# titus-leistner/mmlf

Measured on AMD Instinct MI355X. Metric: 96x96 EPI patches/sec fwd+bwd, bs=512, higher is better.
Workload: dtype f32 via 2 x f16 operand split (22 significant bits per operand, locally scaled; 3 MFMA passes, f32 accumulate)

## Files before the change

### include/mmlf_hip.h

```cpp
#ifndef MMLF_HIP_H
#define MMLF_HIP_H

#include <stddef.h>
#include <stdint.h>

#ifdef __cplusplus
extern "C" {
#endif

#define MMLF_TILE_POSITIONS 256

const char *mmlf_last_error(void);
#define MMLF_ABI_VERSION 10
int mmlf_abi_version(void);

const char *mmlf_build_info(void);
int mmlf_build_is_ablation(void);
int mmlf_conv_cus(void);

enum { MMLF_AUDIT_IN = 0, MMLF_AUDIT_PACKED = 1, MMLF_AUDIT_BIAS = 2, MMLF_AUDIT_OUT = 3, MMLF_AUDIT_REF = 4,
       MMLF_AUDIT_IN_AMAX = 5, MMLF_AUDIT_OUT_AMAX = 6, MMLF_AUDIT_BN_PARTIAL = 7, MMLF_AUDIT_MASK = 8, MMLF_AUDIT_CONV_N = 9 };
int mmlf_audit_conv_h2(int cs_in, int K, int N, int cs_out, int N_store, int out_shift, int cs_ref, int B, int H, int W,
                       int64_t *ends);
enum { MMLF_AUDIT_WG_IN = 0, MMLF_AUDIT_WG_G = 1, MMLF_AUDIT_WG_GW = 2, MMLF_AUDIT_WG_GB = 3, MMLF_AUDIT_WG_WORKSPACE = 4,
       MMLF_AUDIT_WG_IN_AMAX = 5, MMLF_AUDIT_WG_G_AMAX = 6, MMLF_AUDIT_WGRAD_N = 7 };
int mmlf_audit_wgrad_h2(int cs_in, int Cin, int cs_g, int Cout, int g_shift, int B, int H, int W, int64_t *ends);

int64_t mmlf_grid_alloc_positions(int B, int H, int W);
int64_t mmlf_packed_filter_floats(int K, int N);
int64_t mmlf_wgrad_workspace_floats(int Cin, int Cout, int B, int H, int W);

enum { MMLF_VAR_IDENTITY = 0, MMLF_VAR_TRANSPOSE = 1, MMLF_VAR_TRANSPOSE_FLIPH = 2 };

int mmlf_pack_filter(const float *w_oihw, float *packed, int Cout, int Cin, int variant, int dgrad,
                     void *stream);

// ... 63 lines not shown
                        const float *running_var, double eps, float *scale, float *shift, int C,
                        void *stream);
int mmlf_fold_bn_eval(const float *w_oihw, const float *bias, const float *scale, const float *shift,
                      float *w_out, float *bias_out, int Cout, int Cin, void *stream);
int mmlf_bn_stats_finalize(const double *partial, int nblocks, int C, const float *gamma, const float *beta,
                           float *running_mean, float *running_var, double momentum, double eps,
                           float *save_mean, float *save_invstd, float *scale, float *shift,
                           int B, int H, int W, void *stream);
int mmlf_bn_apply_relu(const float *z, int cs_z, int C, const float *scale, const float *shift,
                       float *y, int cs_y, int c_off, int C_store, int B, int H, int W,
                       float *amax_out , void *stream);
int mmlf_bn_apply_relu4(const float *const z[4], int cs_z, int C, const float *const scale[4],
                        const float *const shift[4], float *y, int cs_y, int B, int H, int W,
                        float *amax_out , void *stream);
int mmlf_bn_bwd_reduce(const float *gy, int cs_gy, int c_off, const float *z, int cs_z, int C,
                       const float *scale, const float *shift, const float *gamma,
                       const float *save_mean, const float *save_invstd,
                       float *dgamma, float *dbeta, int accumulate, float *coef,
                       double *partial, int nblocks, int B, int H, int W, void *stream);
int mmlf_bn_bwd_apply(const float *gy, int cs_gy, int c_off, const float *z, int cs_z, int C,
                      const float *scale, const float *shift, const float *save_mean,
                      const float *coef, float *dz, int cs_dz, int B, int H, int W,
                      float *amax_out , void *stream);
int mmlf_relu_bwd_slice(const float *src, int cs_src, int c_off, const float *ref, int cs_ref, int ref_off, int C,
                        float *dst, int cs_dst, int B, int H, int W,
                        float *amax_out , void *stream);
enum { MMLF_AUDIT_SLICE_SRC = 0, MMLF_AUDIT_SLICE_REF = 1, MMLF_AUDIT_SLICE_DST = 2, MMLF_AUDIT_SLICE_AMAX = 3,
       MMLF_AUDIT_SLICE_N = 4 };
int mmlf_audit_relu_bwd_slice(int cs_src, int c_off, int cs_ref, int ref_off, int C, int cs_dst, int B, int H, int W,
                              int64_t *ends);

int mmlf_pack_nchw(const float *nchw, int C, float *grid, int cs, int B, int H, int W,
                   float *amax_out , void *stream);
int mmlf_unpack_nchw(const float *grid, int cs, float *nchw, int C, int B, int H, int W, void *stream);
int mmlf_zero_slack(float *grid, int cs, int B, int H, int W, float *amax, void *stream);
int mmlf_zero_slack4(float *const grid[4], const int cs[4], float *const amax[4], int B, int H, int W, void *stream);

int64_t mmlf_grid_alloc_positions_k3(int B, int H, int W);
int mmlf_zero_slack_k3(float *grid, int cs, int B, int H, int W, float *amax, void *stream);
int mmlf_zero_slack4_k3(float *const grid[4], const int cs[4], float *const amax[4], int B, int H, int W, void *stream);
int64_t mmlf_packed_filter3x3_floats(int K, int N);
int mmlf_pack_filter3x3(const float *w_oihw, float *packed, int Cout, int Cin, int variant, int dgrad, void *stream);
int mmlf_conv3x3(const float *in, int cs_in, int K, const float *packed, const float *bias, int N,
                 float *out, int cs_out, int N_store, int B, int H, int W, int relu, const float *relu_ref, int cs_ref,
                 void *stream);
int64_t mmlf_wgrad3x3_workspace_floats(int Cin, int Cout, int B, int H, int W);
// ... 56 lines not shown
```

### mmlf_amd/_lib.py

```python
import ctypes
import os

_HERE = os.path.dirname(os.path.abspath(__file__))
LIB_PATH = os.environ.get('MMLF_HIP_LIB') or os.path.join(_HERE, 'csrc', 'libmmlf_hip.so')

_vp = ctypes.c_void_p
_i = ctypes.c_int
_i64 = ctypes.c_int64
_d = ctypes.c_double

SIGNATURES = {
    'mmlf_last_error': (ctypes.c_char_p, []),
    'mmlf_abi_version': (_i, []),
    'mmlf_build_info': (ctypes.c_char_p, []),
    'mmlf_build_is_ablation': (_i, []),
    'mmlf_conv_cus': (_i, []),
    'mmlf_audit_conv_h2': (_i, [_i] * 10 + [_vp]),
    'mmlf_audit_wgrad_h2': (_i, [_i] * 8 + [_vp]),
    'mmlf_grid_alloc_positions': (_i64, [_i, _i, _i]),
    'mmlf_packed_filter_floats': (_i64, [_i, _i]),
    'mmlf_wgrad_workspace_floats': (_i64, [_i, _i, _i, _i, _i]),
    'mmlf_pack_filter': (_i, [_vp, _vp, _i, _i, _i, _i, _vp]),
    'mmlf_conv2x2': (_i, [_vp, _i, _i, _vp, _vp, _i, _vp, _i, _i, _i, _i, _i, _i, _i, _i, _i, _vp, _i, _vp]),
    'mmlf_packed_filter_split_bytes': (_i64, [_i, _i]),
# ... 6 lines not shown
    'mmlf_grid_pad_h': (_i, []),
    'mmlf_amax_head': (_i, []),
    'mmlf_amax_shard_stride': (_i, []),
    'mmlf_pack_filter_h2': (_i, [_vp, _vp, _i, _i, _i, _i, _vp]),
    'mmlf_packed_filter_h2_columns': (_i, [_i]),
    'mmlf_pack_filters_h2': (_i, [_vp, _i, _i, _vp]),
    'mmlf_conv2x2_h2': (_i, [_vp, _i, _i, _vp, _vp, _i, _vp, _i, _i, _i, _i, _i, _i, _i, _i, _i, _vp, _i, _vp, _vp, _vp, _vp, _vp, _vp]),
    'mmlf_relu_mask_words': (_i64, [_i, _i, _i]),
    'mmlf_conv2x2_thin_workspace_floats': (_i64, [_i, _i, _i]),
    'mmlf_conv2x2_thin': (_i, [_vp, _i, _i, _vp, _vp, _i, _vp, _i, _i, _i, _i, _i, _i, _i, _i, _i, _vp, _vp, _vp]),
    'mmlf_conv2x2_wgrad_thin_workspace_floats': (_i64, [_i]),
    'mmlf_conv2x2_wgrad_thin': (_i, [_vp, _i, _i, _vp, _i, _i, _i, _vp, _vp, _i, _i, _vp, _i, _i, _i, _vp]),
    'mmlf_conv2x2_blocks': (_i, [_i, _i, _i, _i, _i]),
    'mmlf_bn_stats_finalize': (_i, [_vp, _i, _i, _vp, _vp, _vp, _vp, _d, _d, _vp, _vp, _vp, _vp, _i, _i, _i, _vp]),
    'mmlf_conv2x2_wgrad': (_i, [_vp, _i, _i, _vp, _i, _i, _i, _vp, _vp, _i, _i, _vp, _i, _i, _i, _vp]),
    'mmlf_conv2x2_wgrad_split': (_i, [_vp, _i, _i, _vp, _i, _i, _i, _vp, _vp, _i, _i, _vp, _i, _i, _i, _vp]),
    'mmlf_bn_stats_train': (_i, [_vp, _i, _i, _vp, _vp, _vp, _vp, _d, _d, _vp, _vp, _vp, _vp, _vp, _i, _i, _i, _i, _vp]),
    'mmlf_bn_coeffs_eval': (_i, [_vp, _vp, _vp, _vp, _d, _vp, _vp, _i, _vp]),
    'mmlf_fold_bn_eval': (_i, [_vp, _vp, _vp, _vp, _vp, _vp, _i, _i, _vp]),
    'mmlf_bn_apply_relu': (_i, [_vp, _i, _i, _vp, _vp, _vp, _i, _i, _i, _i, _i, _i, _vp, _vp]),
    'mmlf_bn_apply_relu4': (_i, [_vp, _i, _i, _vp, _vp, _vp, _i, _i, _i, _i, _vp, _vp]),
    'mmlf_bn_bwd_reduce': (_i, [_vp, _i, _i, _vp, _i, _i, _vp, _vp, _vp, _vp, _vp, _vp, _vp, _i, _vp, _vp, _i, _i, _i, _i, _vp]),
    'mmlf_bn_bwd_apply': (_i, [_vp, _i, _i, _vp, _i, _i, _vp, _vp, _vp, _vp, _vp, _i, _i, _i, _i, _vp, _vp]),
    'mmlf_relu_bwd_slice': (_i, [_vp, _i, _i, _vp, _i, _i, _i, _vp, _i, _i, _i, _i, _vp, _vp]),
    'mmlf_audit_relu_bwd_slice': (_i, [_i] * 9 + [_vp]),
    'mmlf_pack_nchw': (_i, [_vp, _i, _vp, _i, _i, _i, _i, _vp, _vp]),
    'mmlf_zero_slack': (_i, [_vp, _i, _i, _i, _i, _vp, _vp]),
    'mmlf_zero_slack4': (_i, [_vp, _vp, _vp, _i, _i, _i, _vp]),
    'mmlf_unpack_nchw': (_i, [_vp, _i, _vp, _i, _i, _i, _i, _vp]),
    'mmlf_head_upr': (_i, [_vp, _vp, _vp, _i, _i, _i, _i, _vp]),
    'mmlf_head_dpp': (_i, [_vp, _vp, _vp, _vp, _vp, _vp, _vp, _i, _i, _i, _i, _vp]),
    'mmlf_head_upr_bwd': (_i, [_vp, _vp, _vp, _vp, _i, _i, _i, _i, _vp]),
    'mmlf_head_dpp_bwd': (_i, [_vp, _vp, _vp, _vp, _vp, _vp, _i, _i, _i, _i, _vp]),
    'mmlf_loss_fwd_bwd': (_i, [_i, _vp, _i, _vp, _vp, _vp, _d, _vp, _vp, _vp, _i, _vp, _i, _i, _i, _vp]),
    'mmlf_loss_multi_scratch_doubles': (_i64, [_i]),
    'mmlf_loss_multi_fwd_bwd': (_i, [_i, _vp, _i, _vp, _i, _vp, _vp, _vp, _d, _vp, _vp, _vp, _i, _vp, _vp, _i, _i, _i, _vp]),
    'mmlf_adam_step': (_i, [_vp, _vp, _vp, _vp, _i64, _d, _d, _d, _d, _i64, _d, _vp]),
    'mmlf_shift_views': (_i, [_vp, _vp, _vp, _vp, _vp, _vp, _vp, _vp, _vp, _vp, _i, _i, _i, _i, _vp]),
    'mmlf_shift_pack': (_i, [_vp, _i, _vp, _i, _vp, _vp, _i, _i, _i, _i, _vp, _vp]),
    'mmlf_lmm_to_discrete': (_i, [_vp, _vp, _vp, _vp, _i, _i, _i, _i64, _vp]),
    'mmlf_patch_gather': (_i, [_vp] * 5 + [_i] * 5 + [_vp] * 12 + [_i, _i, _vp]),
    'mmlf_patch_contrast': (_i, [_vp, _vp, _vp, _vp, _i, _i, _i, _vp]),
    'mmlf_ensamble_reduce': (_i, [_vp, _vp, _vp, _vp, _vp, _vp, _i, _i, _i, _i, _vp]),
    'mmlf_grid_alloc_positions_k3': (_i64, [_i, _i, _i]),
    'mmlf_zero_slack_k3': (_i, [_vp, _i, _i, _i, _i, _vp, _vp]),
    'mmlf_zero_slack4_k3': (_i, [_vp, _vp, _vp, _i, _i, _i, _vp]),
# ... 85 lines not shown
```

### mmlf_amd/csrc/common.h

```cpp
#pragma once
#include <hip/hip_runtime.h>
#include <stdint.h>
#include <stdio.h>
#include <stdarg.h>
#include <mutex>

#define MMLF_TILE 256
#define MMLF_TILE_MAX 512

extern thread_local char g_mmlf_err[512];

static inline int mmlf_fail(const char *fmt, ...)
{
    va_list ap;
    va_start(ap, fmt);
    vsnprintf(g_mmlf_err, sizeof(g_mmlf_err), fmt, ap);
    va_end(ap);
    return 1;
}

#define MMLF_CHECK_ARG(cond, ...)                   \
    do {                                            \
        if (!(cond)) return mmlf_fail(__VA_ARGS__); \
    } while (0)

static inline int mmlf_launch_status(const char *what)
{
    hipError_t e = hipGetLastError();
    if (e != hipSuccess) return mmlf_fail("%s: launch failed: %s", what, hipGetErrorString(e));
    return 0;
}

static inline int current_device()
{
    int d = 0;
    if (hipGetDevice(&d) != hipSuccess || d < 0 || d >= 64) d = 0;
    return d;
}
struct PerDeviceOnce {
    std::once_flag flag[64];
    int status[64] = {};
    template <class F> int run(F &&f)
    {
        const int d = current_device();
        std::call_once(flag[d], [&] { status[d] = f(); });
        return status[d];
    }
};
static inline int mmlf_allow_lds(const void *kernel, size_t bytes, const char *what)
{
    const hipError_t e = hipFuncSetAttribute(kernel, hipFuncAttributeMaxDynamicSharedMemorySize, (int)bytes);
    if (e != hipSuccess)
        return mmlf_fail("%s: hipFuncSetAttribute(MaxDynamicSharedMemorySize = %zu) failed: %s", what, bytes, hipGetErrorString(e));
    return 0;
// ... 99 lines not shown
```

### mmlf_amd/csrc/elementwise.hip

```cpp
#include "common.h"
#include "../../include/mmlf_hip.h"

thread_local char g_mmlf_err[512] = "";

extern "C" const char *mmlf_last_error(void) { return g_mmlf_err; }
extern "C" int mmlf_abi_version(void) { return MMLF_ABI_VERSION; }
extern "C" int64_t mmlf_amax_entries(int B, int H, int W)
{
    if (B <= 0 || H <= 0 || W <= 0) return -1;
    return amax_entries(make_grid(B, H, W));
}
extern "C" int mmlf_grid_pad_w(void) { return GRID_PAD; }
extern "C" int mmlf_grid_pad_h(void) { return GRID_PAD; }
extern "C" int mmlf_amax_head(void) { return MMLF_AMAX_HEAD; }
extern "C" int mmlf_amax_shard_stride(void) { return MMLF_AMAX_SHARD_STRIDE; }
extern "C" int64_t mmlf_grid_alloc_positions(int B, int H, int W)
{
    if (B <= 0 || H <= 0 || W <= 0) return -1;
    return grid_alloc_positions(make_grid(B, H, W));
}
extern "C" int64_t mmlf_grid_alloc_positions_k3(int B, int H, int W)
{
    if (B <= 0 || H <= 0 || W <= 0) return -1;
    return grid_alloc_positions_k3(make_grid(B, H, W));
// ... 286 lines not shown
            for (int k = 0; k < V; ++k) {
                const int c = V * cg + k;
                const float u = fmaf(zz[k], coefs[c], coefs[Cpad + c]);
                if (MODE == 0) {
                    o[k] = fmaxf(u, 0.f);
                } else {
                    const float g = u > 0.f ? gg[k] : 0.f;
                    o[k] = coefs[3 * Cpad + c] * g - coefs[4 * Cpad + c] - coefs[5 * Cpad + c] * (zz[k] - coefs[2 * Cpad + c]);
                }
            }
        }
#pragma unroll
        for (int k = 0; k < V; ++k) mx = fmaxf(mx, fabsf(o[k]));
        float *op = out + (base + x) * cs_out + c_off_out + V * cg;
        if (V * cg + V - 1 < C_store) {
            VecIO<V>::store_nt(op, o);
        } else {
#pragma unroll
            for (int k = 0; k < V; ++k)
                if (V * cg + k < C_store) op[k] = o[k];
        }
    }
    if (amax) mmlf_amax_update_row(mx, amax, row);
    }
}

template <int V>
__global__ __launch_bounds__(256) void relu_slice_rows_kernel(const float *__restrict__ src, int cs_src, int c_off,
                                                              const float *__restrict__ ref, int cs_ref, int ref_off, int C,
                                                              float *__restrict__ dst, int cs_dst, int H, int W,
                                                              float *__restrict__ amax, int nrows)
{
    const int P = W + GRID_PAD, R = H + GRID_PAD;
    const int cvn = cs_dst / V;
    const int dx = 256 / cvn, dc = 256 - dx * cvn;
    for (int row = blockIdx.x; row < nrows; row += gridDim.x) {
        const int y = row % R;
        const size_t base = (size_t)row * P;
        const bool row_in = (y >= 1 && y <= H);
        int x = threadIdx.x / cvn, cg = threadIdx.x - x * cvn;
        float mx = 0.f;
        for (; x < P; x += dx, cg += dc) {
            if (cg >= cvn) { cg -= cvn; ++x; if (x >= P) break; }
            float o[V];
#pragma unroll
            for (int k = 0; k < V; ++k) o[k] = 0.f;
// ... 996 lines not shown
    hipStream_t st = (hipStream_t)stream;
    hipLaunchKernelGGL(bn_reduce_bwd_kernel, dim3(nblocks), dim3(256), 0, st, z, cs_z, gy, cs_gy, c_off,
                       scale, shift, save_mean, save_invstd, C, partial, B, H, W);
    hipLaunchKernelGGL(bn_bwd_finalize_kernel, dim3(C), dim3(64), 0, st, partial, nblocks, C,
                       (double)B * H * W, gamma, save_invstd, dgamma, dbeta, accumulate, coef);
    return mmlf_launch_status("mmlf_bn_bwd_reduce");
}

extern "C" int mmlf_bn_bwd_apply(const float *gy, int cs_gy, int c_off, const float *z, int cs_z, int C,
                                 const float *scale, const float *shift, const float *save_mean, const float *coef,
                                 float *dz, int cs_dz, int B, int H, int W, float *amax_out, void *stream)
{
    MMLF_CHECK_ARG(gy && z && scale && shift && save_mean && coef && dz, "mmlf_bn_bwd_apply: null pointer");
    MMLF_CHECK_ARG(cs_gy % 2 == 0 && c_off % 2 == 0 && c_off >= 0 && cs_z % 4 == 0 && cs_dz % 4 == 0 && C > 0 && C <= cs_z &&
                       C <= cs_dz && c_off + C <= cs_gy,
                   "mmlf_bn_bwd_apply: layout C=%d cs_z=%d cs_dz=%d cs_gy=%d c_off=%d", C, cs_z, cs_dz, cs_gy, c_off);
    MMLF_CHECK_ARG(B > 0 && H > 0 && W > 0, "mmlf_bn_bwd_apply: bad shape B=%d H=%d W=%d", B, H, W);
    const int nrows = B * (H + GRID_PAD);
    hipLaunchKernelGGL((bn_rows_kernel<1, 4>), dim3(nrows), dim3(256), 6 * (cs_dz + 4) * sizeof(float), (hipStream_t)stream, z, cs_z, gy,
                       cs_gy, c_off, scale, shift, save_mean, coef, C, dz, cs_dz, 0, cs_dz, H, W, amax_out, nrows);
    return mmlf_launch_status("mmlf_bn_bwd_apply");
}

static int relu_bwd_slice_args(const char *who, int cs_src, int c_off, int cs_ref, int ref_off, int C, int cs_dst, int B, int H,
                               int W)
{
    MMLF_CHECK_ARG(cs_src > 0 && cs_src % 2 == 0 && c_off % 2 == 0 && c_off >= 0 && cs_dst > 0 && cs_dst % 4 == 0 && C > 0 &&
                       C <= cs_dst && c_off + C <= cs_src && (C + 3) / 4 <= 128 && cs_dst / 4 <= 256,
                   "%s: layout C=%d cs_src=%d c_off=%d cs_dst=%d", who, C, cs_src, c_off, cs_dst);
    MMLF_CHECK_ARG(cs_ref > 0 && cs_ref % 2 == 0 && ref_off % 2 == 0 && ref_off >= 0 && ref_off + C <= cs_ref,
                   "%s: layout C=%d cs_ref=%d ref_off=%d", who, C, cs_ref, ref_off);
    MMLF_CHECK_ARG(B > 0 && H > 0 && W > 0, "%s: bad shape B=%d H=%d W=%d", who, B, H, W);
    return 0;
}

extern "C" int mmlf_relu_bwd_slice(const float *src, int cs_src, int c_off, const float *ref, int cs_ref, int ref_off, int C,
                                   float *dst, int cs_dst, int B, int H, int W, float *amax_out, void *stream)
{
    MMLF_CHECK_ARG(src && ref && dst, "mmlf_relu_bwd_slice: null pointer");
    if (relu_bwd_slice_args("mmlf_relu_bwd_slice", cs_src, c_off, cs_ref, ref_off, C, cs_dst, B, H, W)) return 1;
    const int nrows = B * (H + GRID_PAD);
    hipLaunchKernelGGL((relu_slice_rows_kernel<4>), dim3(nrows), dim3(256), 0, (hipStream_t)stream, src, cs_src, c_off, ref,
                       cs_ref, ref_off, C, dst, cs_dst, H, W, amax_out, nrows);
    return mmlf_launch_status("mmlf_relu_bwd_slice");
}

// ... 313 lines not shown
```

### mmlf_amd/csrc/wgrad.hip

```cpp
#include "conv_device.h"

#ifdef MMLF_BOUNDS_DEBUG
int mmlf_oob_counts_wgrad(unsigned long long *host8, int reset)
{
    if (hipMemcpyFromSymbol(host8, HIP_SYMBOL(g_mmlf_oob), sizeof(unsigned long long) * 8) != hipSuccess) return 1;
    if (reset) {
        const unsigned long long z[8] = {};
        if (hipMemcpyToSymbol(HIP_SYMBOL(g_mmlf_oob), z, sizeof(z)) != hipSuccess) return 1;
    }
    return 0;
}
#endif

struct WgradArgs {
    const float *in;
    const float *g;
    float *part;
    long long NQpad;
    int cs_in, cin, cs_g, g_shift, P, nsplit, nslice, chunks_per_split, nchunks;
    const float *in_amax, *g_amax;
    const float *chunk_scales;
    long long in_bytes, g_bytes, part_floats;
};

// ... 956 lines not shown

extern "C" int64_t mmlf_conv2x2_wgrad_thin_workspace_floats(int Cin)
{
    if (Cin <= 0) return -1;
    return (int64_t)thin_wgrad_waves() * 4 * (Cin + 1) * THIN_MAXN;
}

extern "C" int mmlf_conv2x2_wgrad_thin(const float *in, int cs_in, int Cin, const float *g, int cs_g, int Cout, int g_shift,
                                       float *gw_oihw, float *gb, int variant, int accumulate, float *workspace, int B,
                                       int H, int W, void *stream)
{
    MMLF_CHECK_ARG(in && g && gw_oihw && workspace, "mmlf_conv2x2_wgrad_thin: null pointer");
    MMLF_CHECK_ARG(Cout >= 1 && Cout <= THIN_MAXN && Cout <= cs_g && Cin >= 1 && Cin <= cs_in && cs_in % 4 == 0 && cs_in <= 512,
                   "mmlf_conv2x2_wgrad_thin: Cin=%d Cout=%d cs_in=%d", Cin, Cout, cs_in);
    MMLF_CHECK_ARG(B > 0 && H > 0 && W > 0 && variant >= 0 && variant <= 2, "mmlf_conv2x2_wgrad_thin: bad shape");
    const Grid gr = make_grid(B, H, W);
    MMLF_CHECK_ARG(g_shift >= 0 && g_shift <= gr.P + 1, "mmlf_conv2x2_wgrad_thin: g_shift=%d", g_shift);
    ThinArgs a = {};
    a.in = in; a.g = g; a.wpart = workspace; a.NQ = gr.NQ; a.npos = gr.NQ + gr.P + 2;
    a.cs_in = cs_in; a.C = Cin; a.N = Cout; a.cs_g = cs_g; a.g_shift = g_shift; a.P = gr.P; a.CIP = Cin + 1;
    hipStream_t st = (hipStream_t)stream;
    const int nwaves = thin_wgrad_waves();
    hipLaunchKernelGGL(thin_wgrad_kernel, dim3(nwaves / 4), dim3(256), 0, st, a);
    const int total = 4 * (Cin + 1) * Cout;
    hipLaunchKernelGGL(wgrad_reduce_wave_kernel, dim3((total + 3) / 4), dim3(256), 0, st, workspace, gw_oihw, gb, Cin, Cout,
                       Cin + 1, THIN_MAXN, nwaves, variant, accumulate);
    return mmlf_launch_status("mmlf_conv2x2_wgrad_thin");
}

extern "C" int mmlf_audit_wgrad_h2(int cs_in, int Cin, int cs_g, int Cout, int g_shift, int B, int H, int W,
                                   int64_t *ends )
{
    Wgrad16Cfg c;
    MMLF_CHECK_ARG(B > 0 && H > 0 && W > 0 && ends && Cin > 0 && Cout > 0, "mmlf_audit_wgrad_h2: bad argument");
    const Grid g = make_grid(B, H, W);
    const long long nchunks = g.NQpad / WG_KQ;
    MMLF_CHECK_ARG(wgrad16_cfg(Cin, Cout, nchunks, &c), "mmlf_audit_wgrad_h2: Cout=%d", Cout);
    const long long last_c = (nchunks - 1) * WG_KQ;
    ends[0] = (last_c + g.P + 32 + 1) * cs_in * 4;
    ends[1] = (last_c + g_shift + 31 + 1) * cs_g * 4;
    ends[2] = (int64_t)Cout * Cin * 4 * 4;
    ends[3] = (int64_t)Cout * 4;
    ends[4] = ((int64_t)c.nsplit * 4 * (c.nslice * 16 * c.mb) * (16 * c.nb)
               > wgrad_partial_floats(Cin, Cout) ? -1
               : wgrad_partial_floats(Cin, Cout) + 2 * nchunks + 2) * 4;
    ends[5] = (MMLF_AMAX_HEAD + amax_rows(g)) * 4;
    ends[6] = ends[5];
    return 0;
}

// ... 49 lines not shown
```

### mmlf_amd/engine.py

```python
import os
import threading

import torch

from . import _lib
from ._lib import call, ptr

VAR_IDENTITY, VAR_TRANSPOSE, VAR_TRANSPOSE_FLIPH = 0, 1, 2
BN_BLOCKS = 1024
LOSS_BLOCKS = 1024


def cs_of(c):
    return (c + 7) // 8 * 8


class Geometry:

    def __init__(self, B, H, W, ksize=2):
        self.B, self.H, self.W = B, H, W
        self.ksize = ksize
        self.P, self.R = W + int(_lib.load().mmlf_grid_pad_w()), H + int(_lib.load().mmlf_grid_pad_h())
        self.G = self.P * self.R
        self.NQ = B * self.G
# ... 569 lines not shown
        xmask = None
        for k, spec in enumerate(self.out_blocks):
            if spec.bn is False:
                x, cs_x, xmask = self._block_fwd_relu(geo, spec, VAR_IDENTITY, x, cs_x, k > 0, xmask, p,
                                                      tape['out'] if save else None, packs=packs)
                continue
            x_in = x
            x, cs_x = self._block_fwd(geo, spec, VAR_IDENTITY, x, cs_x, p, train, tape['out'] if save else None, packs=packs,
                                      tracked=tracked)
            if save and not self.batchnorm and k > 0:
                assert tape['out'][-1]['x'] is x_in
                tape['out'][-1].update(x_relu=True, xmask=xmask)
            if not save:
                del tape['out'][:]
        if tracked:
            counts = {}
            for t in tracked:
                counts.setdefault(t.data_ptr(), [t, 0])[1] += 1
            torch._foreach_add_([t for t, _ in counts.values()], [n for _, n in counts.values()])
        out = torch.empty((B, self.oc, H, W), dtype=torch.float32, device=dev)
        call('mmlf_unpack_nchw', ptr(x), cs_x, ptr(out), self.oc, B, H, W, _lib.stream_ptr())
        return out, (tape if save else None)

    def _block_bwd(self, geo, rec, p, grads, gy, cs_gy, c_off, need_dx, after_bn=None, overlap=False, packs=None):
        spec, var = rec['spec'], rec['var']
        dev = gy.device
        ws = _Workspace.get(dev)
        B, H, W, P = geo.B, geo.H, geo.W, geo.P
        C, cs_mid = spec.cout, cs_of(spec.cout)
        x, cs_x, y, z = rec['x'], rec['cs_x'], rec['y'], rec['z']
        pre = spec.prefix
        sp = _lib.stream_ptr
        packs = packs or {}
        k3 = self.ksize == 3

        def packed(name, w):
            pk = packs.get((name, var, True))
            return pk if pk is not None else (pack_filter3 if k3 else pack_filter)(w, var, True)

        x_relu = {}
        if rec.get('x_relu'):
            x_relu = ({'mask_in': rec['xmask']} if rec.get('xmask') is not None and CONV_MODE == 'f16x3'
                      else {'ref': x, 'cs_ref': cs_x})

        got = geo.bufs(([cs_mid] if spec.bn else []) + [cs_mid] + ([cs_x] if need_dx else []), dev)
        dy = got[1 if spec.bn else 0]
        dx = got[-1] if need_dx else None
        if spec.bn:
            coef = torch.empty(3 * C, dtype=torch.float32, device=dev)
            call('mmlf_bn_bwd_reduce', ptr(gy), cs_gy, c_off, ptr(z), cs_mid, C, ptr(rec['scale']), ptr(rec['shift']),
                 ptr(p[f'{pre}.3.weight']), ptr(rec['smean']), ptr(rec['sinv']), ptr(grads[f'{pre}.3.weight']),
                 ptr(grads[f'{pre}.3.bias']), 1, ptr(coef), ptr(ws.partial), BN_BLOCKS, B, H, W, sp())
            if rec.get('eval'):
                coef[C:].zero_()
            dz = got[0]
            call('mmlf_bn_bwd_apply', ptr(gy), cs_gy, c_off, ptr(z), cs_mid, C, ptr(rec['scale']), ptr(rec['shift']),
                 ptr(rec['smean']), ptr(coef), ptr(dz), cs_mid, B, H, W, ptr(dz.absmax), sp())
        else:
            assert c_off == 0 and cs_gy == cs_mid
            dz = gy
        if after_bn:
            after_bn()
        w1, w2 = p[f'{pre}.0.weight'], p[f'{pre}.2.weight']
        if k3:
            wgrad3(geo, y, cs_mid, C, dz, cs_mid, C, grads[f'{pre}.2.weight'], grads[f'{pre}.2.bias'], var, ws.wgrad_ws(geo, C, C))
            conv3(geo, dz, cs_mid, C, packed(f'{pre}.2.weight', w2), None, C, dy, cs_mid, False, ref=y, cs_ref=cs_mid)
            del dz, got
            wgrad3(geo, x, cs_x, spec.cin, dy, cs_mid, C, grads[f'{pre}.0.weight'], grads[f'{pre}.0.bias'], var,
                   ws.wgrad_ws(geo, spec.cin, C))
            if not need_dx:
                return None
            conv3(geo, dy, cs_mid, C, packed(f'{pre}.0.weight', w1), None, spec.cin, dx, cs_x, False)
            return dx
        wgrad(geo, y, cs_mid, C, dz, cs_mid, C, P + 1, grads[f'{pre}.2.weight'], grads[f'{pre}.2.bias'], var,
              ws.wgrad_ws(geo, C, C))
        pk = packed(f'{pre}.2.weight', w2)
        if rec.get('ymask') is not None and CONV_MODE == 'f16x3':
            conv(geo, dz, cs_mid, C, pk, None, C, dy, cs_mid, 0, H + 1, W + 1, False, mask_in=rec['ymask'])
        else:
            conv(geo, dz, cs_mid, C, pk, None, C, dy, cs_mid, 0, H + 1, W + 1, False, ref=y, cs_ref=cs_mid)
        del dz, got
        if overlap and need_dx:
            pk = packed(f'{pre}.0.weight', w1)
            conv(geo, dy, cs_mid, C, pk, None, spec.cin, dx, cs_x, P + 1, H, W, False, **x_relu)
            main = torch.cuda.current_stream()
            ready = main.record_event()
            with torch.cuda.stream(ws.side):
                ws.side.wait_event(ready)
                wgrad(geo, x, cs_x, spec.cin, dy, cs_mid, C, 0, grads[f'{pre}.0.weight'], grads[f'{pre}.0.bias'],
                      var, ws.wgrad_ws(geo, spec.cin, C, side=True), side=True)
                done = ws.side.record_event()
            return dx, done, (x, dy)
        wgrad(geo, x, cs_x, spec.cin, dy, cs_mid, C, 0, grads[f'{pre}.0.weight'], grads[f'{pre}.0.bias'], var,
              ws.wgrad_ws(geo, spec.cin, C))
        if not need_dx:
            return None
        pk = packed(f'{pre}.0.weight', w1)
        conv(geo, dy, cs_mid, C, pk, None, spec.cin, dx, cs_x, P + 1, H, W, False, **x_relu)
        return dx

    def backward(self, p, tape, grad_output, grads, on_done=None):
        geo = tape['geo']
        dev = grad_output.device
        _Workspace.get(dev).enter_stream()
        B, H, W = geo.B, geo.H, geo.W
        cs = cs_of(self.oc)
        g = geo.buf(cs, dev)
        call('mmlf_pack_nchw', ptr(grad_output.contiguous()), self.oc, ptr(g), cs, B, H, W, ptr(g.absmax),
             _lib.stream_ptr())
        cs_g = cs
        recs = tape['out']
        main = torch.cuda.current_stream()
        pending = None

        def settle():
            nonlocal pending
            if pending is not None:
                main.wait_event(pending[0])
                if on_done:
                    on_done(pending[1])
                pending = None

        while recs:
            rec = recs.pop()
            wide = OVERLAP_WGRAD and rec['spec'].cin >= 128 and self.ksize == 2
            res = self._block_bwd(geo, rec, p, grads, g, cs_g, 0, True, after_bn=settle, overlap=wide, packs=tape.get('packs'))
            settle()
            if wide:
                g, ev, keep = res
                pending = (ev, rec['spec'].prefix, keep)
            else:
                g = res
                if on_done:
                    on_done(rec['spec'].prefix)
            cs_g = rec['cs_x']
        for s in reversed(range(4)):
            recs = tape['streams'][s]
            if s == 2:
                settle()
            gs, cs_s, off = g, cs_g, s * self.chs
            if not self.batchnorm:
                cs_s, off = cs_of(self.chs), 0
                gs = geo.buf(cs_s, dev)
                relu_bwd_slice(geo, g, cs_g, s * self.chs, tape['concat'], cs_g, s * self.chs, self.chs, gs, cs_s)
            while recs:
                rec = recs.pop()
                gs = self._block_bwd(geo, rec, p, grads, gs, cs_s, off, need_dx=bool(recs), packs=tape.get('packs'))
                cs_s, off = rec['cs_x'], 0
            if on_done and s in (2, 0):
# ... 2 lines not shown
```

Before: 1126.

## Fold thin head conv backward into preceding block's BN backward kernels

For the final block's first conv, which has at most two output channels, the backward pass no longer runs a separate dgrad conv and thin wgrad. The previous block's BN backward reduce and apply kernels instead recompute the incoming gradient on the fly from the head's dy and filter taps. The reduce kernel also accumulates the head weight and bias gradients in double precision, and a shared finish kernel reduces them. This removes a full-size intermediate gradient buffer write and read plus extra launches, at the cost of heavier, register-hungry BN kernels that redo a small 4-tap dot product per channel in both passes.

```diff
diff --git a/include/mmlf_hip.h b/include/mmlf_hip.h
--- a/include/mmlf_hip.h
+++ b/include/mmlf_hip.h
@@ -11,7 +11,7 @@
 #define MMLF_TILE_POSITIONS 256
 
 const char *mmlf_last_error(void);
-#define MMLF_ABI_VERSION 10
+#define MMLF_ABI_VERSION 11
 int mmlf_abi_version(void);
 
 const char *mmlf_build_info(void);
@@ -121,6 +121,19 @@
                       const float *scale, const float *shift, const float *save_mean,
                       const float *coef, float *dz, int cs_dz, int B, int H, int W,
                       float *amax_out , void *stream);
+int64_t mmlf_bn_head_bwd_workspace_floats(int C, int nblocks);
+int mmlf_bn_head_bwd_reduce(const float *dy_head, int cs_dy, const float *w_head, int N, int variant, const float *z,
+                            int cs_z, int C, const float *scale, const float *shift, const float *gamma,
+                            const float *save_mean, const float *save_invstd, float *dgamma, float *dbeta,
+                            int accumulate, float *coef, double *partial, int nblocks, float *gw_head, float *gb_head,
+                            int accumulate_head, float *workspace, int B, int H, int W, void *stream);
+int mmlf_bn_head_bwd_apply(const float *dy_head, int cs_dy, const float *w_head, int N, int variant, const float *z,
+                           int cs_z, int C, const float *scale, const float *shift, const float *save_mean,
+                           const float *coef, float *dz, int cs_dz, int B, int H, int W,
+                           float *amax_out , void *stream);
+enum { MMLF_AUDIT_HEAD_DY = 0, MMLF_AUDIT_HEAD_W = 1, MMLF_AUDIT_HEAD_Z = 2, MMLF_AUDIT_HEAD_DZ = 3, MMLF_AUDIT_HEAD_AMAX = 4,
+       MMLF_AUDIT_HEAD_PARTIAL = 5, MMLF_AUDIT_HEAD_WORKSPACE = 6, MMLF_AUDIT_HEAD_N = 7 };
+int mmlf_audit_bn_head_bwd(int cs_dy, int N, int cs_z, int C, int cs_dz, int nblocks, int B, int H, int W, int64_t *ends);
 int mmlf_relu_bwd_slice(const float *src, int cs_src, int c_off, const float *ref, int cs_ref, int ref_off, int C,
                         float *dst, int cs_dst, int B, int H, int W,
                         float *amax_out , void *stream);
diff --git a/mmlf_amd/_lib.py b/mmlf_amd/_lib.py
--- a/mmlf_amd/_lib.py
+++ b/mmlf_amd/_lib.py
@@ -52,6 +52,11 @@
     'mmlf_bn_apply_relu4': (_i, [_vp, _i, _i, _vp, _vp, _vp, _i, _i, _i, _i, _vp, _vp]),
     'mmlf_bn_bwd_reduce': (_i, [_vp, _i, _i, _vp, _i, _i, _vp, _vp, _vp, _vp, _vp, _vp, _vp, _i, _vp, _vp, _i, _i, _i, _i, _vp]),
     'mmlf_bn_bwd_apply': (_i, [_vp, _i, _i, _vp, _i, _i, _vp, _vp, _vp, _vp, _vp, _i, _i, _i, _i, _vp, _vp]),
+    'mmlf_bn_head_bwd_workspace_floats': (_i64, [_i, _i]),
+    'mmlf_bn_head_bwd_reduce': (_i, [_vp, _i, _vp, _i, _i, _vp, _i, _i, _vp, _vp, _vp, _vp, _vp, _vp, _vp, _i, _vp, _vp, _i, _vp, _vp,
+                                     _i, _vp, _i, _i, _i, _vp]),
+    'mmlf_bn_head_bwd_apply': (_i, [_vp, _i, _vp, _i, _i, _vp, _i, _i, _vp, _vp, _vp, _vp, _vp, _i, _i, _i, _i, _vp, _vp]),
+    'mmlf_audit_bn_head_bwd': (_i, [_i] * 9 + [_vp]),
     'mmlf_relu_bwd_slice': (_i, [_vp, _i, _i, _vp, _i, _i, _i, _vp, _i, _i, _i, _i, _vp, _vp]),
     'mmlf_audit_relu_bwd_slice': (_i, [_i] * 9 + [_vp]),
     'mmlf_pack_nchw': (_i, [_vp, _i, _vp, _i, _i, _i, _i, _vp, _vp]),
diff --git a/mmlf_amd/csrc/common.h b/mmlf_amd/csrc/common.h
--- a/mmlf_amd/csrc/common.h
+++ b/mmlf_amd/csrc/common.h
@@ -30,6 +30,9 @@
     if (e != hipSuccess) return mmlf_fail("%s: launch failed: %s", what, hipGetErrorString(e));
     return 0;
 }
+
+void thin_wgrad_finish(const float *part, float *gw_oihw, float *gb, int Cin, int Cout, int nsplit, int variant, int accumulate,
+                       hipStream_t st);
 
 static inline int current_device()
 {
diff --git a/mmlf_amd/csrc/elementwise.hip b/mmlf_amd/csrc/elementwise.hip
--- a/mmlf_amd/csrc/elementwise.hip
+++ b/mmlf_amd/csrc/elementwise.hip
@@ -332,6 +332,235 @@
         }
     }
     if (amax) mmlf_amax_update_row(mx, amax, row);
+    }
+}
+
+constexpr int HEAD_MAXN = 2;
+
+template <int NO>
+__device__ __forceinline__ void head_filter_regs(const float *__restrict__ wh, int variant, int C, int c0, float (&w)[4][4][NO])
+{
+#pragma unroll
+    for (int e = 0; e < 4; ++e)
+#pragma unroll
+        for (int t = 0; t < 4; ++t)
+#pragma unroll
+            for (int o = 0; o < NO; ++o)
+                w[e][t][o] = c0 + e < C ? wh[((size_t)o * C + c0 + e) * 4 + master_tap<2>(t, variant)] : 0.f;
+}
+
+template <int NO>
+__device__ __forceinline__ void head_dy_taps(const float *__restrict__ dyh, int cs_dy, size_t p, int P, float (&d)[4][NO])
+{
+    const int offs[4] = {0, 1, P, P + 1};
+#pragma unroll
+    for (int t = 0; t < 4; ++t) {
+        const float *q = dyh + (p - offs[t]) * cs_dy;
+        if constexpr (NO == 2) {
+            const float2 v = *reinterpret_cast<const float2 *>(q);
+            d[t][0] = v.x; d[t][1] = v.y;
+        } else {
+            d[t][0] = q[0];
+        }
+    }
+}
+
+template <int NO>
+__device__ __forceinline__ float head_gy(const float (&w)[4][NO], const float (&d)[4][NO])
+{
+    float g = 0.f;
+#pragma unroll
+    for (int t = 0; t < 4; ++t)
+#pragma unroll
+        for (int o = 0; o < NO; ++o) g = fmaf(w[t][o], d[t][o], g);
+    return g;
+}
+
+template <int NO>
+__global__ __launch_bounds__(256)
+void bn_head_reduce_bwd_kernel(const float *__restrict__ z, int cs_z, const float *__restrict__ dyh, int cs_dy,
+                               const float *__restrict__ wh, int variant, const float *__restrict__ scale,
+                               const float *__restrict__ shift, const float *__restrict__ mean,
+                               const float *__restrict__ invstd, int C, double *__restrict__ partial,
+                               float *__restrict__ wpart, int B, int H, int W)
+{
+    constexpr int V = 4;
+    const int P = W + GRID_PAD, R = H + GRID_PAD;
+    const int cvn = (C + V - 1) / V, ppi = 256 / cvn;
+    const int tid = threadIdx.x;
+    const int pl = tid / cvn, cg = tid - pl * cvn;
+    const bool active = pl < ppi;
+    __shared__ double red[2][256][V];
+    float wr[V][4][NO], sc[V], sh[V], mu[V], iv[V];
+    head_filter_regs<NO>(wh, variant, C, V * cg, wr);
+#pragma unroll
+    for (int e = 0; e < V; ++e) {
+        const int c = V * cg + e;
+        const bool in = c < C;
+        sc[e] = in ? scale[c] : 0.f; sh[e] = in ? shift[c] : 0.f;
+        mu[e] = in ? mean[c] : 0.f;  iv[e] = in ? invstd[c] : 0.f;
+    }
+    double s0[V], s1[V], dw[V][4][NO];
+#pragma unroll
+    for (int e = 0; e < V; ++e) {
+        s0[e] = 0; s1[e] = 0;
+#pragma unroll
+        for (int t = 0; t < 4; ++t)
+#pragma unroll
+            for (int o = 0; o < NO; ++o) dw[e][t][o] = 0;
+    }
+    const int nrows = B * H;
+    const bool z_aligned = (reinterpret_cast<uintptr_t>(z) & 15) == 0 && (cs_z & 3) == 0;
+    constexpr int U = 2;
+    for (int row = blockIdx.x; row < nrows; row += gridDim.x) {
+        const int b = row / H, y = row - b * H + 1;
+        const size_t base = ((size_t)(b * R + y) * P + 1);
+        for (int x0 = pl; active && x0 < W; x0 += U * ppi) {
+            float zz[U][V], d[U][4][NO];
+#pragma unroll
+            for (int k = 0; k < U; ++k) {
+                const int x = x0 + k * ppi < W ? x0 + k * ppi : x0;
+                VecIO<V>::load_nt(z + (base + x) * cs_z + V * cg, zz[k], z_aligned);
+                head_dy_taps<NO>(dyh, cs_dy, base + x, P, d[k]);
+            }
+#pragma unroll
+            for (int k = 0; k < U; ++k) {
+                if (x0 + k * ppi >= W) break;
+                double dd[4][NO];
+#pragma unroll
+                for (int t = 0; t < 4; ++t)
+#pragma unroll
+                    for (int o = 0; o < NO; ++o) dd[t][o] = (double)d[k][t][o];
+#pragma unroll
+                for (int e = 0; e < V; ++e) {
+                    const float u = fmaf(zz[k][e], sc[e], sh[e]);
+                    const float g = u > 0.f ? head_gy<NO>(wr[e], d[k]) : 0.f;
+                    const double r = (double)fmaxf(u, 0.f);
+                    s0[e] += g;
+                    s1[e] += (double)g * (double)((zz[k][e] - mu[e]) * iv[e]);
+#pragma unroll
+                    for (int t = 0; t < 4; ++t)
+#pragma unroll
+                        for (int o = 0; o < NO; ++o) dw[e][t][o] = fma(r, dd[t][o], dw[e][t][o]);
+                }
+            }
+        }
+    }
+    double bs[NO];
+#pragma unroll
+    for (int o = 0; o < NO; ++o) bs[o] = 0;
+    const long long NQ = (long long)B * R * P;
+    for (long long q = (long long)blockIdx.x * 256 + tid; q < NQ; q += (long long)gridDim.x * 256)
+#pragma unroll
+        for (int o = 0; o < NO; ++o) bs[o] += (double)dyh[(size_t)q * cs_dy + o];
+
+#pragma unroll
+    for (int e = 0; e < V; ++e) { red[0][tid][e] = s0[e]; red[1][tid][e] = s1[e]; }
+    __syncthreads();
+    if (tid < cvn) {
+#pragma unroll
+        for (int e = 0; e < V; ++e) {
+            double a0 = 0, a1 = 0;
+            for (int p = 0; p < ppi; ++p) { a0 += red[0][p * cvn + tid][e]; a1 += red[1][p * cvn + tid][e]; }
+            const int c = V * tid + e;
+            if (c < C) {
+                partial[((size_t)blockIdx.x * 2 + 0) * C + c] = a0;
+                partial[((size_t)blockIdx.x * 2 + 1) * C + c] = a1;
+            }
+        }
+    }
+    const int CIP = C + 1;
+    const size_t plane = (size_t)4 * CIP * HEAD_MAXN;
+    float *hi = wpart + (size_t)blockIdx.x * 2 * plane, *lo = hi + plane;
+#pragma unroll
+    for (int t = 0; t < 4; ++t) {
+        __syncthreads();
+#pragma unroll
+        for (int e = 0; e < V; ++e)
+#pragma unroll
+            for (int o = 0; o < NO; ++o) red[o][tid][e] = dw[e][t][o];
+        __syncthreads();
+        if (tid < cvn) {
+#pragma unroll
+            for (int e = 0; e < V; ++e) {
+                const int c = V * tid + e;
+#pragma unroll
+                for (int o = 0; o < NO; ++o) {
+                    double a = 0;
+                    for (int p = 0; p < ppi; ++p) a += red[o][p * cvn + tid][e];
+                    if (c < C) {
+                        const size_t i = ((size_t)t * CIP + c) * HEAD_MAXN + o;
+                        hi[i] = (float)a;
+                        lo[i] = (float)(a - (double)(float)a);
+                    }
+                }
+            }
+        }
+    }
+    __syncthreads();
+#pragma unroll
+    for (int o = 0; o < NO; ++o) red[0][tid][o] = bs[o];
+    __syncthreads();
+    if (tid < 64) {
+#pragma unroll
+        for (int o = 0; o < NO; ++o) {
+            double a = red[0][tid][o] + red[0][tid + 64][o] + red[0][tid + 128][o] + red[0][tid + 192][o];
+#pragma unroll
+            for (int k = 32; k > 0; k >>= 1) a += __shfl_xor(a, k);
+            if (tid == 0) {
+                hi[(size_t)C * HEAD_MAXN + o] = (float)a;
+                lo[(size_t)C * HEAD_MAXN + o] = (float)(a - (double)(float)a);
+            }
+        }
+    }
+}
+
+template <int NO>
+__global__ __launch_bounds__(256)
+void bn_head_rows_bwd_kernel(const float *__restrict__ z, int cs_z, const float *__restrict__ dyh, int cs_dy,
+                             const float *__restrict__ wh, int variant, const float *__restrict__ scale,
+                             const float *__restrict__ shift, const float *__restrict__ mean,
+                             const float *__restrict__ coef, int C, float *__restrict__ out, int cs_out, int H, int W,
+                             float *__restrict__ amax, int nrows)
+{
+    constexpr int V = 4;
+    const int P = W + GRID_PAD, R = H + GRID_PAD;
+    const int cvn = cs_out / V, ppi = 256 / cvn;
+    const int pl = threadIdx.x / cvn, cg = threadIdx.x - pl * cvn;
+    float wr[V][4][NO], sc[V], sh[V], mu[V], k1[V], k2[V], k3[V];
+    head_filter_regs<NO>(wh, variant, C, V * cg, wr);
+#pragma unroll
+    for (int e = 0; e < V; ++e) {
+        const int c = V * cg + e;
+        const bool in = c < C;
+        sc[e] = in ? scale[c] : 0.f; sh[e] = in ? shift[c] : 0.f; mu[e] = in ? mean[c] : 0.f;
+        k1[e] = in ? coef[c] : 0.f;  k2[e] = in ? coef[C + c] : 0.f; k3[e] = in ? coef[2 * C + c] : 0.f;
+    }
+    for (int row = blockIdx.x; row < nrows; row += gridDim.x) {
+        const int y = row % R;
+        const size_t base = (size_t)row * P;
+        const bool row_in = (y >= 1 && y <= H);
+        float mx = 0.f;
+        for (int x = pl; pl < ppi && x < P; x += ppi) {
+            float o[V];
+#pragma unroll
+            for (int k = 0; k < V; ++k) o[k] = 0.f;
+            if (row_in && x >= 1 && x <= W && V * cg < C) {
+                float zz[V], d[4][NO];
+                VecIO<V>::load_nt(z + (base + x) * cs_z + V * cg, zz);
+                head_dy_taps<NO>(dyh, cs_dy, base + x, P, d);
+#pragma unroll
+                for (int k = 0; k < V; ++k) {
+                    const float u = fmaf(zz[k], sc[k], sh[k]);
+                    const float g = u > 0.f ? head_gy<NO>(wr[k], d) : 0.f;
+                    o[k] = k1[k] * g - k2[k] - k3[k] * (zz[k] - mu[k]);
+                }
+            }
+#pragma unroll
+            for (int k = 0; k < V; ++k) mx = fmaxf(mx, fabsf(o[k]));
+            VecIO<V>::store_nt(out + (base + x) * cs_out + V * cg, o);
+        }
+        if (amax) mmlf_amax_update_row(mx, amax, row);
     }
 }
 
@@ -1374,6 +1603,87 @@
     return mmlf_launch_status("mmlf_bn_bwd_apply");
 }
 
+static int bn_head_bwd_args(const char *who, int cs_dy, int N, int variant, int cs_z, int C, int B, int H, int W)
+{
+    MMLF_CHECK_ARG(N >= 1 && N <= HEAD_MAXN && cs_dy >= HEAD_MAXN && cs_dy % 2 == 0 && variant >= 0 && variant <= 2,
+                   "%s: head N=%d cs_dy=%d variant=%d (N <= 2, even cs_dy >= 2)", who, N, cs_dy, variant);
+    MMLF_CHECK_ARG(cs_z % 4 == 0 && C > 0 && C <= cs_z && (C + 3) / 4 <= 128, "%s: layout C=%d cs_z=%d", who, C, cs_z);
+    MMLF_CHECK_ARG(B > 0 && H > 0 && W > 0, "%s: bad shape B=%d H=%d W=%d", who, B, H, W);
+    const Grid g = make_grid(B, H, W);
+    MMLF_CHECK_ARG(g.NQpad + 2 * g.P + 64 < (1ll << 31), "%s: batch x image too large", who);
+    return 0;
+}
+
+extern "C" int64_t mmlf_bn_head_bwd_workspace_floats(int C, int nblocks)
+{
+    if (C <= 0 || nblocks <= 0) return -1;
+    return (int64_t)nblocks * 2 * 4 * (C + 1) * HEAD_MAXN;
+}
+
+extern "C" int mmlf_bn_head_bwd_reduce(const float *dy_head, int cs_dy, const float *w_head, int N, int variant, const float *z,
+                                       int cs_z, int C, const float *scale, const float *shift, const float *gamma,
+                                       const float *save_mean, const float *save_invstd, float *dgamma, float *dbeta,
+                                       int accumulate, float *coef, double *partial, int nblocks, float *gw_head,
+                                       float *gb_head, int accumulate_head, float *workspace, int B, int H, int W,
+                                       void *stream)
+{
+    MMLF_CHECK_ARG(dy_head && w_head && z && scale && shift && save_mean && save_invstd && coef && partial && gw_head &&
+                       workspace,
+                   "mmlf_bn_head_bwd_reduce: null pointer");
+    MMLF_CHECK_ARG((reinterpret_cast<uintptr_t>(dy_head) & 7) == 0, "mmlf_bn_head_bwd_reduce: dy_head is not 8-byte aligned");
+    if (bn_head_bwd_args("mmlf_bn_head_bwd_reduce", cs_dy, N, variant, cs_z, C, B, H, W)) return 1;
+    MMLF_CHECK_ARG(nblocks > 0 && nblocks <= 4096, "mmlf_bn_head_bwd_reduce: nblocks=%d", nblocks);
+    hipStream_t st = (hipStream_t)stream;
+    if (N == 1)
+        hipLaunchKernelGGL((bn_head_reduce_bwd_kernel<1>), dim3(nblocks), dim3(256), 0, st, z, cs_z, dy_head, cs_dy, w_head,
+                           variant, scale, shift, save_mean, save_invstd, C, partial, workspace, B, H, W);
+    else
+        hipLaunchKernelGGL((bn_head_reduce_bwd_kernel<2>), dim3(nblocks), dim3(256), 0, st, z, cs_z, dy_head, cs_dy, w_head,
+                           variant, scale, shift, save_mean, save_invstd, C, partial, workspace, B, H, W);
+    hipLaunchKernelGGL(bn_bwd_finalize_kernel, dim3(C), dim3(64), 0, st, partial, nblocks, C,
+                       (double)B * H * W, gamma, save_invstd, dgamma, dbeta, accumulate, coef);
+    thin_wgrad_finish(workspace, gw_head, gb_head, C, N, 2 * nblocks, variant, accumulate_head, st);
+    return mmlf_launch_status("mmlf_bn_head_bwd_reduce");
+}
+
+extern "C" int mmlf_bn_head_bwd_apply(const float *dy_head, int cs_dy, const float *w_head, int N, int variant, const float *z,
+                                      int cs_z, int C, const float *scale, const float *shift, const float *save_mean,
+                                      const float *coef, float *dz, int cs_dz, int B, int H, int W, float *amax_out,
+                                      void *stream)
+{
+    MMLF_CHECK_ARG(dy_head && w_head && z && scale && shift && save_mean && coef && dz, "mmlf_bn_head_bwd_apply: null pointer");
+    MMLF_CHECK_ARG((reinterpret_cast<uintptr_t>(dy_head) & 7) == 0, "mmlf_bn_head_bwd_apply: dy_head is not 8-byte aligned");
+    if (bn_head_bwd_args("mmlf_bn_head_bwd_apply", cs_dy, N, variant, cs_z, C, B, H, W)) return 1;
+    MMLF_CHECK_ARG(cs_dz % 4 == 0 && C <= cs_dz && cs_dz / 4 <= 256, "mmlf_bn_head_bwd_apply: layout C=%d cs_dz=%d", C, cs_dz);
+    const int nrows = B * (H + GRID_PAD);
+    hipStream_t st = (hipStream_t)stream;
+    if (N == 1)
+        hipLaunchKernelGGL((bn_head_rows_bwd_kernel<1>), dim3(nrows), dim3(256), 0, st, z, cs_z, dy_head, cs_dy, w_head, variant,
+                           scale, shift, save_mean, coef, C, dz, cs_dz, H, W, amax_out, nrows);
+    else
+        hipLaunchKernelGGL((bn_head_rows_bwd_kernel<2>), dim3(nrows), dim3(256), 0, st, z, cs_z, dy_head, cs_dy, w_head, variant,
+                           scale, shift, save_mean, coef, C, dz, cs_dz, H, W, amax_out, nrows);
+    return mmlf_launch_status("mmlf_bn_head_bwd_apply");
+}
+
+extern "C" int mmlf_audit_bn_head_bwd(int cs_dy, int N, int cs_z, int C, int cs_dz, int nblocks, int B, int H, int W,
+                                      int64_t *ends )
+{
+    MMLF_CHECK_ARG(ends && nblocks > 0, "mmlf_audit_bn_head_bwd: bad argument");
+    if (bn_head_bwd_args("mmlf_audit_bn_head_bwd", cs_dy, N, 0, cs_z, C, B, H, W)) return 1;
+    MMLF_CHECK_ARG(cs_dz % 4 == 0 && C <= cs_dz, "mmlf_audit_bn_head_bwd: layout C=%d cs_dz=%d", C, cs_dz);
+    const Grid g = make_grid(B, H, W);
+    const long long q_last = ((long long)(B - 1) * g.R + H) * g.P + W;
+    ends[MMLF_AUDIT_HEAD_DY] = ((g.NQ - 1) * cs_dy + N) * 4;
+    ends[MMLF_AUDIT_HEAD_W] = (int64_t)N * C * 4 * 4;
+    ends[MMLF_AUDIT_HEAD_Z] = (q_last * cs_z + (C + 3) / 4 * 4) * 4;
+    ends[MMLF_AUDIT_HEAD_DZ] = g.NQ * cs_dz * 4;
+    ends[MMLF_AUDIT_HEAD_AMAX] = (MMLF_AMAX_HEAD + (long long)B * g.R) * 4;
+    ends[MMLF_AUDIT_HEAD_PARTIAL] = (int64_t)nblocks * 2 * C * 8;
+    ends[MMLF_AUDIT_HEAD_WORKSPACE] = mmlf_bn_head_bwd_workspace_floats(C, nblocks) * 4;
+    return 0;
+}
+
 static int relu_bwd_slice_args(const char *who, int cs_src, int c_off, int cs_ref, int ref_off, int C, int cs_dst, int B, int H,
                                int W)
 {
diff --git a/mmlf_amd/csrc/wgrad.hip b/mmlf_amd/csrc/wgrad.hip
--- a/mmlf_amd/csrc/wgrad.hip
+++ b/mmlf_amd/csrc/wgrad.hip
@@ -1002,10 +1002,16 @@
     hipStream_t st = (hipStream_t)stream;
     const int nwaves = thin_wgrad_waves();
     hipLaunchKernelGGL(thin_wgrad_kernel, dim3(nwaves / 4), dim3(256), 0, st, a);
+    thin_wgrad_finish(workspace, gw_oihw, gb, Cin, Cout, nwaves, variant, accumulate, st);
+    return mmlf_launch_status("mmlf_conv2x2_wgrad_thin");
+}
+
+void thin_wgrad_finish(const float *part, float *gw_oihw, float *gb, int Cin, int Cout, int nsplit, int variant, int accumulate,
+                       hipStream_t st)
+{
     const int total = 4 * (Cin + 1) * Cout;
-    hipLaunchKernelGGL(wgrad_reduce_wave_kernel, dim3((total + 3) / 4), dim3(256), 0, st, workspace, gw_oihw, gb, Cin, Cout,
-                       Cin + 1, THIN_MAXN, nwaves, variant, accumulate);
-    return mmlf_launch_status("mmlf_conv2x2_wgrad_thin");
+    hipLaunchKernelGGL(wgrad_reduce_wave_kernel, dim3((total + 3) / 4), dim3(256), 0, st, part, gw_oihw, gb, Cin, Cout,
+                       Cin + 1, THIN_MAXN, nsplit, variant, accumulate);
 }
 
 extern "C" int mmlf_audit_wgrad_h2(int cs_in, int Cin, int cs_g, int Cout, int g_shift, int B, int H, int W,
diff --git a/mmlf_amd/engine.py b/mmlf_amd/engine.py
--- a/mmlf_amd/engine.py
+++ b/mmlf_amd/engine.py
@@ -615,9 +615,10 @@
         call('mmlf_unpack_nchw', ptr(x), cs_x, ptr(out), self.oc, B, H, W, _lib.stream_ptr())
         return out, (tape if save else None)
 
-    def _block_bwd(self, geo, rec, p, grads, gy, cs_gy, c_off, need_dx, after_bn=None, overlap=False, packs=None):
+    def _block_bwd(self, geo, rec, p, grads, gy, cs_gy, c_off, need_dx, after_bn=None, overlap=False, packs=None,
+                   head=None, fold_conv1=False):
         spec, var = rec['spec'], rec['var']
-        dev = gy.device
+        dev = rec['y'].device
         ws = _Workspace.get(dev)
         B, H, W, P = geo.B, geo.H, geo.W, geo.P
         C, cs_mid = spec.cout, cs_of(spec.cout)
@@ -636,10 +637,31 @@
             x_relu = ({'mask_in': rec['xmask']} if rec.get('xmask') is not None and CONV_MODE == 'f16x3'
                       else {'ref': x, 'cs_ref': cs_x})
 
+        need_dx = need_dx and not fold_conv1
         got = geo.bufs(([cs_mid] if spec.bn else []) + [cs_mid] + ([cs_x] if need_dx else []), dev)
         dy = got[1 if spec.bn else 0]
         dx = got[-1] if need_dx else None
-        if spec.bn:
+        if spec.bn and head is not None:
+            assert not rec.get('eval') and not k3
+            coef = torch.empty(3 * C, dtype=torch.float32, device=dev)
+            dz = got[0]
+            hws = ws.scratch('bn_head_bwd', int(_lib.load().mmlf_bn_head_bwd_workspace_floats(C, BN_BLOCKS)))
+            hd = (ptr(head['dy']), head['cs_dy'], ptr(head['w']), head['N'], head['var'])
+            if CHECK_EXTENTS:
+                import ctypes
+                e = (ctypes.c_int64 * 7)()
+                call('mmlf_audit_bn_head_bwd', head['cs_dy'], head['N'], cs_mid, C, cs_mid, BN_BLOCKS, B, H, W, e)
+                _check_extents(f'bn_head_bwd C={C} N={head["N"]} B={B} {H}x{W}', e,
+                               {'dy_head': (e[0], head['dy'], 0), 'w_head': (e[1], head['w'], 0), 'z': (e[2], z, 0),
+                                'dz': (e[3], dz, 0), 'amax': (e[4], dz.absmax, 0), 'partial': (e[5], ws.partial, 0),
+                                'workspace': (e[6], hws, 0)})
+            call('mmlf_bn_head_bwd_reduce', *hd, ptr(z), cs_mid, C, ptr(rec['scale']), ptr(rec['shift']),
+                 ptr(p[f'{pre}.3.weight']), ptr(rec['smean']), ptr(rec['sinv']), ptr(grads[f'{pre}.3.weight']),
+                 ptr(grads[f'{pre}.3.bias']), 1, ptr(coef), ptr(ws.partial), BN_BLOCKS, ptr(head['gw']), ptr(head['gb']), 1,
+                 ptr(hws), B, H, W, sp())
+            call('mmlf_bn_head_bwd_apply', *hd, ptr(z), cs_mid, C, ptr(rec['scale']), ptr(rec['shift']), ptr(rec['smean']),
+                 ptr(coef), ptr(dz), cs_mid, B, H, W, ptr(dz.absmax), sp())
+        elif spec.bn:
             coef = torch.empty(3 * C, dtype=torch.float32, device=dev)
             call('mmlf_bn_bwd_reduce', ptr(gy), cs_gy, c_off, ptr(z), cs_mid, C, ptr(rec['scale']), ptr(rec['shift']),
                  ptr(p[f'{pre}.3.weight']), ptr(rec['smean']), ptr(rec['sinv']), ptr(grads[f'{pre}.3.weight']),
@@ -673,6 +695,9 @@
         else:
             conv(geo, dz, cs_mid, C, pk, None, C, dy, cs_mid, 0, H + 1, W + 1, False, ref=y, cs_ref=cs_mid)
         del dz, got
+        if fold_conv1:
+            return {'dy': dy, 'cs_dy': cs_mid, 'w': w1, 'N': C, 'var': var, 'gw': grads[f'{pre}.0.weight'],
+                    'gb': grads[f'{pre}.0.bias']}
         if overlap and need_dx:
             pk = packed(f'{pre}.0.weight', w1)
             conv(geo, dy, cs_mid, C, pk, None, spec.cin, dx, cs_x, P + 1, H, W, False, **x_relu)
@@ -692,6 +717,15 @@
         conv(geo, dy, cs_mid, C, pk, None, spec.cin, dx, cs_x, P + 1, H, W, False, **x_relu)
         return dx
 
+    def _head_folds(self, rec, below):
+        spec = rec['spec']
+        if self.ksize != 2 or spec.bn is not None or not below:
+            return False
+        if not (spec.cout <= THIN_MAX_N and spec.cin >= THIN_MIN_K and rec['cs_x'] <= 512):
+            return False
+        prev = below[-1]
+        return bool(prev['spec'].bn) and not prev.get('eval') and prev['spec'].cout == spec.cin
+
     def backward(self, p, tape, grad_output, grads, on_done=None):
         geo = tape['geo']
         dev = grad_output.device
@@ -709,15 +743,24 @@
         def settle():
             nonlocal pending
             if pending is not None:
-                main.wait_event(pending[0])
+                if pending[0] is not None:
+                    main.wait_event(pending[0])
                 if on_done:
                     on_done(pending[1])
                 pending = None
 
+        head = None
         while recs:
             rec = recs.pop()
+            if self._head_folds(rec, recs):
+                head = self._block_bwd(geo, rec, p, grads, g, cs_g, 0, True, packs=tape.get('packs'), fold_conv1=True)
+                pending = (None, rec['spec'].prefix, ())
+                g, cs_g = None, rec['cs_x']
+                continue
             wide = OVERLAP_WGRAD and rec['spec'].cin >= 128 and self.ksize == 2
-            res = self._block_bwd(geo, rec, p, grads, g, cs_g, 0, True, after_bn=settle, overlap=wide, packs=tape.get('packs'))
+            res = self._block_bwd(geo, rec, p, grads, g, cs_g, 0, True, after_bn=settle, overlap=wide, packs=tape.get('packs'),
+                                  head=head)
+            head = None
             settle()
             if wide:
                 g, ev, keep = res
```

After: 1135 (median of 6 runs). About the same (+0.8%).
